# kkahatapitiya/Coarse-Fine-Networks

Hardware: AMD Instinct MI355X
Metric: clips/sec (fwd+bwd+SGD) x3d_fine X3D-M T=256x224x224 (higher is better)
Workload: dtype f32; 1 GPU; x3d_fine X3D-M train step (fwd+loss+bwd+SGD), 8x3x256x224x224 clips per GPU, random-init weights; clips_per_gpu=8, frames=256, parallelism=dp1, launch=eager

## Files before the change

coarse-fine-networks_amd/cfn_hip/ops.py:

```python
import torch
from torch.autograd import Function
from torch.autograd.function import once_differentiable

import ctypes
import threading

from . import call, call_try, check, query, last_error, ACT_NONE, ACT_RELU, ACT_SWISH, ACT_SIGMOID


_scratch_epoch = [0]


class _ZeroArena(object):
    CHUNK = 1 << 20

    def __init__(self):
        self.buf, self.off, self.epoch = {}, {}, _scratch_epoch[0]

    def take(self, numel, dev):
        if self.epoch != _scratch_epoch[0]:
            self.buf, self.off, self.epoch = {}, {}, _scratch_epoch[0]
        numel_al = (numel + 1) & ~1
        key = (dev.type, dev.index)
        if key not in self.buf or self.off[key] + numel_al > self.buf[key].numel():
            self.buf[key] = torch.zeros(max(self.CHUNK, numel_al), dtype=torch.float64, device=dev)
            self.off[key] = 0
        o = self.off[key]
        self.off[key] = o + numel_al
        return self.buf[key][o:o + numel]


class _GradCast(object):

    def __init__(self):
        self._reset()
        self.last_total = 0

    def _reset(self):
        self.cur, self.live, self.scheduled, self.seen, self.task = {}, [], False, set(), None

    def begin(self):
        tid = torch._C._current_graph_task_id()
        if tid != self.task:
            if self.live:
                self.flush()
            self._reset()
            self.task = tid

    def first_use(self, w):
        if id(w) in self.seen:
            return False
        self.seen.add(id(w))
        return True

    def take(self, numel, shape, dev):
        al = (numel + 3) & ~3
        key = (dev.type, dev.index)
        ch = self.cur.get(key)
        if ch is None or ch['off'] + al > ch['f64'].numel():
            size = max(int(self.last_total * 1.05) + 1024, al, 1 << 16)
            ch = {'f64': torch.zeros(size, dtype=torch.float64, device=dev),
                  'f32': torch.empty(size, dtype=torch.float32, device=dev), 'off': 0, 'done': 0}
            self.cur[key] = ch
            self.live.append(ch)
        o = ch['off']
        ch['off'] = o + al
        if not self.scheduled:
            torch.autograd.Variable._execution_engine.queue_callback(self._end_of_backward)
            self.scheduled = True
        return ch['f64'][o:o + numel], ch['f32'][o:o + numel].view(shape)

    def flush(self):
        for ch in self.live:
            if ch['off'] > ch['done']:
                ch['f32'][ch['done']:ch['off']].copy_(ch['f64'][ch['done']:ch['off']])
                ch['done'] = ch['off']

    def _end_of_backward(self):
        self.flush()
        self.last_total = max(sum(ch['off'] for ch in self.live), 1)
        self._reset()


class _PerThread(threading.local):

    def __init__(self):
        self.arena = _ZeroArena()
# ... 344 lines not shown


class _DwConvT5(Function):

    @staticmethod
    def forward(ctx, x, w, want_stats, out_dtype=None):
        x = check(x, torch.float32).contiguous()
        N, C, T, H, W = x.shape
        y = torch.empty_like(x, dtype=out_dtype or x.dtype)
        s = q = None
        if want_stats:
            s, q = _f64(N, C, x.device), _f64(N, C, x.device)
        w2 = w.reshape(C, 5).contiguous()
        call('cfn_dwconv_t5_fwd' + _sfx(y), x, w2, y, s, q, N, C, T, H * W)
        ctx.save_for_backward(x, w2, y)
        ctx.wshape = tuple(w.shape)
        ctx.wparam = w
        if not want_stats:
            return y, None, None
        return y, s, q

    @staticmethod
    @once_differentiable
    def backward(ctx, gy, gs, gq):
        x, w2, y = ctx.saved_tensors
        N, C, T, H, W = x.shape
        gy = torch.zeros_like(y) if gy is None else gy.contiguous()
        gs, gq = _opt(gs), _opt(gq)
        gx = gw = None
        want_x, want_w = ctx.needs_input_grad[0], ctx.needs_input_grad[1]
        if want_x:
            gx = torch.empty_like(x)
        if want_w:
            g64, fin = _gw_buffers(ctx.wparam, C, 5, x.device)
        fused = want_x and want_w and call_try('cfn_dwconv_t5_bwd_fused' + _sfx(y), gy, y, gs, gq, w2, x, gx, g64, N, C, T, H * W)
        if not fused:
            if want_x:
                call('cfn_dwconv_t5_bwd_data' + _sfx(y), gy, y, gs, gq, w2, gx, N, C, T, H * W)
            if want_w:
                call('cfn_dwconv_t5_bwd_weight' + _sfx(y), gy, y, gs, gq, x, g64, N, C, T, H * W)
        if want_w:
            gw = fin()
        return gx, gw, None, None


def dwconv_t5(x, w, stats=True, out_dtype=None):
    return _DwConvT5.apply(x, w, stats, out_dtype)


class _StemConv(Function):

    @staticmethod
    def forward(ctx, x, w):
        x = check(x).contiguous()
        N, Ci, T, H, W = x.shape
        Co = w.shape[0]
        Ho, Wo = (H + 2 - 3) // 2 + 1, (W + 2 - 3) // 2 + 1
        y = torch.empty(N, Co, T, Ho, Wo, dtype=torch.float32, device=x.device)
        w2 = w.reshape(Co, Ci * 9).contiguous()
        call('cfn_stem_conv_fwd', x, w2, y, N, Ci, Co, T, H, W)
        ctx.save_for_backward(x)
        ctx.wshape = tuple(w.shape)
        ctx.wparam = w
        return y

    @staticmethod
    @once_differentiable
    def backward(ctx, gy):
        (x,) = ctx.saved_tensors
        N, Ci, T, H, W = x.shape
        Co = ctx.wshape[0]
        gw = None
        if ctx.needs_input_grad[1]:
            g64, fin = _gw_buffers(ctx.wparam, Co, Ci * 9, x.device)
            call('cfn_stem_conv_bwd_weight', gy.contiguous(), x, g64, N, Ci, Co, T, H, W)
            gw = fin()
        return None, gw


def stem_conv(x, w):
    return _StemConv.apply(x, w)


from .u8clips import clip_lut


def _u8_args(frames, lengths, lut):
    if frames.dtype != torch.uint8 or frames.dim() != 5 or frames.shape[4] != 3:
        raise RuntimeError('uint8 frames of shape (N, T, H, W, 3) expected, got %s %s' % (frames.dtype, tuple(frames.shape)))
    if lut.dtype != torch.float32 or lut.numel() != 3 * 256:
        raise RuntimeError('a (3, 256) fp32 table expected (ops.clip_lut), got %s %s' % (lut.dtype, tuple(lut.shape)))
    if lengths is not None:
        if lengths.numel() != frames.shape[0]:
            raise RuntimeError('one length per clip expected: %d clips, lengths %s' % (frames.shape[0], tuple(lengths.shape)))
        lengths = lengths.to(torch.int32).contiguous()
    return frames.contiguous(), lengths, lut.contiguous()


def clip_u8_to_f32(frames, lut, lengths=None):
    frames, lengths, lut = _u8_args(frames, lengths, lut)
    N, T, H, W, _ = frames.shape
    x = torch.empty(N, 3, T, H, W, dtype=torch.float32, device=frames.device)
    call('cfn_clip_u8_to_f32', frames, lut, lengths, x, N, T, H, W)
    return x


class _StemConvU8(Function):

    @staticmethod
    def forward(ctx, frames, lengths, lut, w):
        frames, lengths, lut = _u8_args(frames, lengths, lut)
        N, T, H, W, Ci = frames.shape
        Co = w.shape[0]
        Ho, Wo = (H + 2 - 3) // 2 + 1, (W + 2 - 3) // 2 + 1
        y = torch.empty(N, Co, T, Ho, Wo, dtype=torch.float32, device=frames.device)
        w2 = w.reshape(Co, Ci * 9).contiguous()
        if not call_try('cfn_stem_conv_u8_fwd', frames, lut, lengths, w2, y, N, Ci, Co, T, H, W):
            call('cfn_stem_conv_fwd', clip_u8_to_f32(frames, lut, lengths), w2, y, N, Ci, Co, T, H, W)
        ctx.save_for_backward(frames, lengths, lut)
        ctx.wshape = tuple(w.shape)
        ctx.wparam = w
        return y

    @staticmethod
    @once_differentiable
    def backward(ctx, gy):
        frames, lengths, lut = ctx.saved_tensors
        N, T, H, W, Ci = frames.shape
        Co = ctx.wshape[0]
        gw = None
        if ctx.needs_input_grad[3]:
            g64, fin = _gw_buffers(ctx.wparam, Co, Ci * 9, frames.device)
            gy = gy.contiguous()
            if not call_try('cfn_stem_conv_u8_bwd_weight', gy, frames, lut, lengths, g64, N, Ci, Co, T, H, W):
                call('cfn_stem_conv_bwd_weight', gy, clip_u8_to_f32(frames, lut, lengths), g64, N, Ci, Co, T, H, W)
            gw = fin()
        return None, None, None, gw


def stem_conv_u8(frames, lengths, lut, w):
    return _StemConvU8.apply(frames, lengths, lut, w)


from . import u8aug

_AUG_TABLES = {}
_AUG_TABLES_MAX = 256


def aug_tables(box, size, device):
    cs = tuple(int(v) for v in box.detach().reshape(-1, 4)[:, 2].cpu().tolist())
    device = torch.device(device)
    key = (cs, int(size), device.type, device.index)
    hit = _AUG_TABLES.get(key)
    if hit is None:
        if any(c <= 0 or c > 4 * int(size) for c in cs):
            raise RuntimeError('crop_resize_flip_u8: crop extents %s into %d: 1 <= c <= 4 * size expected (the kernel takes tables of up '
                               'to %d taps; there is no CPU fallback)' % (sorted(set(cs)), size, u8aug.MAX_TAPS))
        bounds, coef = u8aug.batch_tables(cs, size)
        hit = (bounds.to(device), coef.to(device))
        if len(_AUG_TABLES) >= _AUG_TABLES_MAX:
            _AUG_TABLES.clear()
        _AUG_TABLES[key] = hit
    return hit


# ... 1185 lines not shown
```

coarse-fine-networks_amd/x3d_coarse.py:

```python
import threading

import torch
import torch.nn as nn
import torch.nn.functional as F

from cfn_hip import ops, ACT_NONE, ACT_RELU, ACT_SWISH, ACT_SIGMOID
from interp1d import Interp1d
from x3d_fine import (SubBatchNorm3d, Swish, Bottleneck, Deferred, conv3x3x3, conv1x1x1, _count,
                      get_inplanes, get_blocks)
import x3d_fine

FUSION_HW = 7


def _o():
    if x3d_fine.USE_TORCH_OPS:
        from cfn_hip import torchlib
        return torchlib.TorchOps
    return ops


def _w5(conv1d):
    w = conv1d.weight
    return w.view(w.shape[0], w.shape[1], 1, 1, 1)
# ... 248 lines not shown
        return mix(bias, self.conv_at, ACT_NONE), mix(scale, self.conv_at2, ACT_SIGMOID)

    def forward(self, inp):
        x, bias, scale = inp
        h = x.shape[3]
        zero = lambda v: torch.zeros(v.shape[1], device=v.device)
        down = lambda v: (v[:, :, :, ::v.shape[3] // FUSION_HW, ::v.shape[4] // FUSION_HW].contiguous(), zero(v))
        c7, m7 = self.forward7([down(v) for v in bias], [down(v) for v in scale])
        return _upsample(c7, h), _upsample(m7, h)


class _ZeroGradFor(torch.autograd.Function):

    @staticmethod
    def forward(ctx, t, param):
        ctx.meta = (tuple(param.shape), param.dtype, param.device)
        return t.view_as(t)

    @staticmethod
    def backward(ctx, g):
        shape, dt, dev = ctx.meta
        return g, torch.zeros(shape, dtype=dt, device=dev)


class GridPoolLayer(nn.Module):

    def __init__(self, ratio, depth):
        super(GridPoolLayer, self).__init__()
        self.ratio = 4
        self.depth = depth
        self.conv1 = nn.Conv3d(depth, depth, kernel_size=(3, 3, 3), stride=(self.ratio // 2, 2, 2), padding=1)
        self.bn1 = SubBatchNorm3d(num_splits=1, num_features=depth, affine=True)
        self.conv2 = nn.Conv3d(depth, depth, kernel_size=(3, 3, 3), stride=(self.ratio // 2, 2, 2), padding=1)
        self.bn2 = SubBatchNorm3d(num_splits=1, num_features=depth, affine=True)
        self.conv3 = nn.Conv3d(depth, 1, kernel_size=(1, 3, 3), stride=(1, 2, 2), padding=(0, 1, 1))
        self.relu = nn.ReLU(inplace=True)
        self.sigmoid = nn.Sigmoid()

    def _conv_bn(self, x, conv, bn, A, B, act):
        n = x.shape[0]
        st = tuple(conv.stride)
        y, s, q = _o().conv3d_dense(x, conv.weight, (3, 3, 3), st, (1, 1, 1), A, B, act, stats=self.training)
        A2, B2 = (bn.fold_op if x3d_fine.USE_TORCH_OPS else bn.fold)(s, q, _count(y), n)
        if not self.training:
            return y, A2, torch.addcmul(B2, A2, conv.bias.to(B2.dtype).view(1, -1))
        with torch.no_grad():
            bn.split_bn.running_mean.view(-1, bn.num_features).add_(conv.bias.view(1, -1), alpha=bn.momentum)
        return y, A2, _ZeroGradFor.apply(B2, conv.bias)

    def saliency(self, x):
        y1, A1, B1 = self._conv_bn(x, self.conv1, self.bn1, None, None, ACT_NONE)
        y2, A2, B2 = self._conv_bn(y1, self.conv2, self.bn2, A1, B1, ACT_RELU)
        y3, _, _ = _o().conv3d_dense(y2, self.conv3.weight, (1, 3, 3), (1, 2, 2), (0, 1, 1), A2, B2, ACT_RELU, stats=False)
        g = _o().pool_hw(y3, 1, 1)
        return g.view(g.shape[0], g.shape[2])

    @staticmethod
    def cdf(g, bias=None):
        return _o().grid_cdf(g, bias)

    def forward(self, inp):
        x = inp.materialize() if isinstance(inp, Deferred) else inp
        gx_out = self.cdf(self.saliency(x), self.conv3.bias)
        return _o().time_sample(x, gx_out), gx_out


def GridUnpool(inp, return_aux=False):
    x, gx, is_logit = inp
    ratio = 4
    b, k = gx.shape
    mid = torch.arange(k, device=gx.device).to(torch.float32)
    mid = (mid / (k - 1.)).view(1, -1).repeat(b, 1)
    gx_inv, ind = Interp1d().forward(gx, mid, mid, None, return_index=True)
    if is_logit:
        y = _o().time_sample(x.unsqueeze(3), gx_inv).squeeze(3)
    else:
        y = _o().time_resize(_o().time_sample(x, gx_inv), x.shape[2] * ratio)
    if return_aux:
        return y, gx_inv, ind
    return y


class ResNet(x3d_fine.ResNet):

    def __init__(self, block, layers, block_inplanes, n_input_channels=3, feat_depth={}, conv1_t_size=7,
                 conv1_t_stride=1, shortcut_type='B', widen_factor=1.0, dropout=0.5, n_classes=400, base_bn_splits=8,
                 task='class', extract_feat=False, t_pool=None, learnedMixing=False, isMixing=False, act_dtype=None):
        self.feat_depth, self.learnedMixing, self.isMixing, self.t_pool = feat_depth, learnedMixing, isMixing, t_pool
        nn.Module.__init__(self)
        planes = [(int(x * widen_factor), int(y * widen_factor)) for x, y in block_inplanes]
        if t_pool == 'avg':
            self.pool_1 = nn.AvgPool3d((4, 1, 1), stride=(4, 1, 1))
        elif t_pool == 'max':
            self.pool_1 = nn.MaxPool3d((4, 1, 1), stride=(4, 1, 1))
        elif t_pool == 'grid':
            self.pool_1 = GridPoolLayer(ratio=4, depth=planes[0][1])
        x3d_fine.ResNet.__init__(self, block, layers, block_inplanes, n_input_channels=n_input_channels,
                                 shortcut_type=shortcut_type, widen_factor=widen_factor, dropout=dropout,
                                 n_classes=n_classes, base_bn_splits=base_bn_splits, task=task,
                                 extract_feat=extract_feat, _skip_module_init=True, act_dtype=act_dtype)
        self.rw2 = RewightLayer(planes[0][1], planes[0][1], feat_depth['layer1'], 56)
        self.rw3 = RewightLayer(planes[1][1], planes[1][1], feat_depth['layer2'], 28)
        self.rw4 = RewightLayer(planes[2][1], planes[2][1], feat_depth['layer3'], 14)
        self.rw5 = RewightLayer(planes[3][1], planes[3][1], feat_depth['layer4'], 7)
        self.rw6 = RewightLayer(157, 157, feat_depth['conv5'], 7, pool=True)
        if self.isMixing:
            self.mix2 = MixingLayer(planes[0][1], learned=learnedMixing, index=0)
            self.mix3 = MixingLayer(planes[1][1], learned=learnedMixing, index=1)
            self.mix4 = MixingLayer(planes[2][1], learned=learnedMixing, index=2)
            self.mix5 = MixingLayer(planes[3][1], learned=learnedMixing, index=3)
        self.gauss = Gaussian(ratio=1)
        for m in self.modules():
            if isinstance(m, nn.Conv3d):
                nn.init.kaiming_normal_(m.weight, mode='fan_out', nonlinearity='relu')

    def replace_logits(self, n_classes):
        dev = self.fc1.weight.device
        self.fc2 = nn.Linear(2048, n_classes).to(dev)
        self.rw6 = RewightLayer(n_classes, n_classes, self.feat_depth['conv5'], 7, pool=True).to(dev)

    def forward(self, inp):
        x, feat, feat_masks, i, meta = inp
        tl = x.shape[2]
        x = self.layer1(self._stem(x))
        if self.act_dtype != torch.float32:
            x = (x.materialize() if isinstance(x, Deferred) else x).float()
        if self.t_pool == 'grid':
            x, gx = self.pool_1(x)
            GX = self.gauss([meta, feat_masks, gx, tl])
        else:
            if self.t_pool == 'stride':
                x = x[:, :, ::4].contiguous()
            elif self.t_pool in ('avg', 'max'):
                x = ops.time_pool(x.materialize() if isinstance(x, Deferred) else x, self.t_pool, 4)
            GX = self.gauss([meta, feat_masks, x, None])
        b2 = x.shape[0]
        levels = (('layer1', self.rw2), ('layer2', self.rw3), ('layer3', self.rw4), ('layer4', self.rw5))
        stages = (None, self.layer2, self.layer3, self.layer4)
        with _row_bank(b2, self._bias_groups(levels, feat, b2)):
            return self._fuse(x, feat, feat_masks, GX, gx if self.t_pool == 'grid' else None, b2, levels, stages)

    def _bias_groups(self, levels, feat, b2):
        rws = [m for _, m in levels] + ([] if self.extract_feat else [self.rw6])
        groups = []
        for m in rws:
            groups += [[m.fc1.bias]] + ([[m.fc3.bias]] if m.g_channels is not None else [])
        for (k, m) in list(levels) + ([] if self.extract_feat else [('conv5', self.rw6)]):
            if feat[k].shape[0] == b2:
                groups.append([m.at1.bias])
        if self.isMixing:
            groups += [[m.fc2.bias for _, m in levels], [m.fc4.bias for _, m in levels]]
            for mix in (self.mix2, self.mix3, self.mix4, self.mix5):
                if mix.learned:
                    groups += [[mix.conv_at.bias], [mix.conv_at2.bias]]
        else:
            for _, m in levels:
                groups += [[m.fc2.bias], [m.fc4.bias]]
        return groups

    def _fuse(self, x, feat, feat_masks, GX, gx, b2, levels, stages):
        if self.isMixing:
            rw = [m.forward7(feat[k], b2, feat_masks, GX, True) for k, m in levels]
            rb, rs = MixingLayer.prepare([r[0] for r in rw]), MixingLayer.prepare([r[1] for r in rw])
            for li, mix in enumerate((self.mix2, self.mix3, self.mix4, self.mix5)):
                if stages[li] is not None:
                    x = stages[li](x)
# ... 31 lines not shown
```

coarse-fine-networks_amd/x3d_fine.py:

```python
import os

import torch
import torch.nn as nn
import torch.nn.functional as F

from cfn_hip import ops, ACT_NONE, ACT_RELU, ACT_SWISH
from cfn_hip.u8clips import U8Clips

USE_TORCH_OPS = os.environ.get('CFN_USE_TORCH_OPS', '0') == '1'


class Deferred(object):
    __slots__ = ('raw', 'A', 'B', 'act')

    def __init__(self, raw, A, B, act):
        self.raw, self.A, self.B, self.act = raw, A, B, act

    @property
    def shape(self):
        return self.raw.shape

    def materialize(self):
        return ops.affine_act(self.raw, self.A, self.B, self.act)

# ... 198 lines not shown
            super(ResNet, self).__init__()
        block_inplanes = [(int(x * widen_factor), int(y * widen_factor)) for x, y in block_inplanes]
        self.index = 0
        self.base_bn_splits = base_bn_splits
        self.task = task
        self.extract_feat = extract_feat
        self.global_tower = global_tower
        self.t_downsample = t_downsample
        self.act_dtype = {None: torch.float32, 'f32': torch.float32, 'fp32': torch.float32, torch.float32: torch.float32,
                          'bf16': torch.bfloat16, torch.bfloat16: torch.bfloat16,
                          'fp16': torch.float16, 'f16': torch.float16, torch.float16: torch.float16}[act_dtype]
        self.in_planes = block_inplanes[0][1]

        self.conv1_s = nn.Conv3d(n_input_channels, self.in_planes, kernel_size=(1, 3, 3), stride=(1, 2, 2),
                                 padding=(0, 1, 1), bias=False)
        self.conv1_t = nn.Conv3d(self.in_planes, self.in_planes, kernel_size=(5, 1, 1), stride=(1, 1, 1),
                                 padding=(2, 0, 0), bias=False, groups=self.in_planes)
        self.bn1 = SubBatchNorm3d(num_splits=base_bn_splits, num_features=self.in_planes, affine=True)
        self.relu = nn.ReLU(inplace=True)
        self.layer1 = self._make_layer(block, block_inplanes[0], layers[0], shortcut_type, stride=2)
        self.layer2 = self._make_layer(block, block_inplanes[1], layers[1], shortcut_type, stride=2)
        self.layer3 = self._make_layer(block, block_inplanes[2], layers[2], shortcut_type, stride=2)
        self.layer4 = self._make_layer(block, block_inplanes[3], layers[3], shortcut_type, stride=2)
        self.conv5 = nn.Conv3d(block_inplanes[3][1], block_inplanes[3][0], kernel_size=(1, 1, 1), stride=(1, 1, 1),
                               padding=(0, 0, 0), bias=False)
        self.bn5 = SubBatchNorm3d(num_splits=base_bn_splits, num_features=block_inplanes[3][0], affine=True)
        if task == 'class':
            self.avgpool = nn.AdaptiveAvgPool3d((1, 1, 1))
        elif task == 'loc':
            self.avgpool = nn.AdaptiveAvgPool3d((None, 1, 1))
        self.fc1 = nn.Conv3d(block_inplanes[3][0], 2048, bias=False, kernel_size=1, stride=1)
        self.fc2 = nn.Linear(2048, n_classes)
        self.dropout = nn.Dropout(dropout)

        for m in self.modules():
            if isinstance(m, nn.Conv3d):
                nn.init.kaiming_normal_(m.weight, mode='fan_out', nonlinearity='relu')

    def _make_layer(self, block, planes, blocks, shortcut_type, stride=1):
        downsample = None
        if stride != 1 or self.in_planes != planes[1]:
            if shortcut_type == 'A':
                downsample = ('A', planes[1], stride)
            else:
                downsample = nn.Sequential(
                    conv1x1x1(self.in_planes, planes[1], stride, t_downsample=self.t_downsample),
                    SubBatchNorm3d(num_splits=self.base_bn_splits, num_features=planes[1], affine=True))
        layers = [block(in_planes=self.in_planes, planes=planes, stride=stride, downsample=downsample,
                        index=self.index, base_bn_splits=self.base_bn_splits, t_downsample=self.t_downsample)]
        self.in_planes = planes[1]
        self.index += 1
        for _ in range(1, blocks):
            layers.append(block(self.in_planes, planes, index=self.index, base_bn_splits=self.base_bn_splits,
                                t_downsample=self.t_downsample))
            self.index += 1
        self.index = 0
        for blk in layers[:-1]:
            blk.split_out = True
        return nn.Sequential(*layers)

    def replace_logits(self, n_classes):
        self.fc2 = nn.Linear(2048, n_classes).to(self.fc1.weight.device)

    def update_bn_splits_long_cycle(self, long_cycle_bn_scale):
        for m in self.modules():
            if isinstance(m, SubBatchNorm3d):
                m.num_splits = self.base_bn_splits * long_cycle_bn_scale
                m.split_bn = nn.BatchNorm3d(num_features=m.num_features * m.num_splits, affine=False).to(m.weight.device)
        return self.base_bn_splits * long_cycle_bn_scale

    def aggregate_sub_bn_stats(self):
        count = 0
        for m in self.modules():
            if isinstance(m, SubBatchNorm3d):
                m.aggregate_stats()
                count += 1
        return count

    def set_input_norm(self, mean, std, norm_value=255):
        lut = ops.clip_lut(mean, std, norm_value).to(self.conv1_s.weight.device)
        self.register_buffer('input_lut', lut, persistent=False)
        return self

    def _conv1_s(self, x):
        if not isinstance(x, U8Clips):
            return ops.stem_conv(x, self.conv1_s.weight)
        lut = getattr(self, 'input_lut', None)
        if lut is None:
            raise RuntimeError('the model was handed uint8 frames (U8Clips) but does not know how to normalise them: call '
                               'set_input_norm(mean, std) first (e.g. CHARADES_MEAN / CHARADES_STD)')
        if x.frames.dim() != 5:
            raise RuntimeError('U8Clips of shape (N, T, H, W, 3) expected (flatten_crops() a collated batch), got %s'
                               % (tuple(x.frames.shape),))
        return ops.stem_conv_u8(x.frames, x.lengths, lut, self.conv1_s.weight)

    def _stem(self, x):
        y = self._conv1_s(x)
        y, s, q = ops.dwconv_t5(y, self.conv1_t.weight, stats=self.training, out_dtype=self.act_dtype)
        A, B = self.bn1.fold(s, q, _count(y), y.shape[0])
        return Deferred(y, A, B, ACT_RELU)

    def _head(self, x):
        n = x.shape[0]
        y5, s5, q5 = ops.pwconv(x, self.conv5.weight, stats=self.training)
        A5, B5 = self.bn5.fold(s5, q5, _count(y5), n)
        if self.task == 'class':
            pooled = ops.pool_hw(y5, 1, 1, A5, B5, ACT_RELU).mean(dim=2, keepdim=True)
        else:
            pooled = ops.pool_hw(y5, 1, 1, A5, B5, ACT_RELU)
        if self.extract_feat:
            return pooled
        f1, _, _ = ops.pwconv(pooled, self.fc1.weight, stats=False)
        one = torch.ones(n, f1.shape[1], device=f1.device)
        z = ops.affine_act(f1, one, torch.zeros_like(one), ACT_RELU)
        z = self.dropout(z)
        out, _, _ = ops.pwconv(z, self.fc2.weight.view(self.fc2.weight.shape[0], -1, 1, 1, 1), stats=False)
        out = out.squeeze(4).squeeze(3) + self.fc2.bias.view(1, -1, 1)
        return out

    def forward(self, inp):
        x, masks = inp
        x = self._stem(x)
        feat_g = {}
        for i, layer in enumerate((self.layer1, self.layer2, self.layer3, self.layer4), start=1):
            x = layer(x)
            if self.global_tower:
                feat_g['layer%d' % i] = ops.pool_hw(x, 7, 7)
        if self.global_tower:
            n = x.shape[0]
            y5, s5, q5 = ops.pwconv(x, self.conv5.weight, stats=self.training)
            A5, B5 = self.bn5.fold(s5, q5, _count(y5), n)
            feat_g['conv5'] = ops.pool_hw(y5, 7, 7, A5, B5, ACT_RELU)
            return feat_g, masks
        return self._head(x)


def replace_logits(self, n_classes):
    self.fc2 = nn.Linear(2048, n_classes)


def get_inplanes(version):
    planes = {'S': [(54, 24), (108, 48), (216, 96), (432, 192)],
              'M': [(54, 24), (108, 48), (216, 96), (432, 192)],
              'XL': [(72, 32), (162, 72), (306, 136), (630, 280)]}
    return planes[version]


def get_blocks(version):
    blocks = {'S': [3, 5, 11, 7], 'M': [3, 5, 11, 7], 'XL': [5, 10, 25, 15]}
    return blocks[version]


def generate_model(x3d_version, **kwargs):
    return ResNet(Bottleneck, get_blocks(x3d_version), get_inplanes(x3d_version), **kwargs)
```

include/cfn_hip.h:

```cpp
#ifndef CFN_HIP_H
#define CFN_HIP_H
#ifdef __cplusplus
extern "C" {
#endif

const char* cfn_last_error(void);
const char* cfn_version(void);
int cfn_device_info(int* cus, int* lds_per_cu, char* name, int name_len);

int cfn_prof_enable(int family, int on);
int cfn_prof_collect(int family, double* total_ms, long* launches, double* total_bytes);

int cfn_dwconv3d_fwd(const float* x, const double* A, const double* B, int act, const float* w, float* y, double* sum,
                     double* sumsq, int N, int C, int T, int Hi, int Wi, int stride, void* stream);
int cfn_dwconv3d_bwd_data(const float* gy, const float* y, const double* gsum, const double* gsumsq, const float* w,
                          const float* x, const double* A, const double* B, int act, float* gx, double* gA, double* gB,
                          int N, int C, int T, int Hi, int Wi, int stride, void* stream);
int cfn_dwconv3d_bwd_weight(const float* gy, const float* y, const double* gsum, const double* gsumsq, const float* x,
                            const double* A, const double* B, int act, double* gw, int N, int C, int T, int Hi, int Wi,
                            int stride, void* stream);
int cfn_dwconv3d_bwd_fused(const float* gy, const float* y, const double* gsum, const double* gsumsq, const float* w,
                           const float* x, const double* A, const double* B, int act, float* gx, double* gA, double* gB,
                           double* gw, int N, int C, int T, int H, int W, void* stream);
int cfn_dwconv3d_bwd_fused_s2(const float* gy, const float* y, const double* gsum, const double* gsumsq, const float* w,
                              const float* x, const double* A, const double* B, int act, float* gx, double* gA, double* gB,
                              double* gw, int N, int C, int T, int H, int W, void* stream);

int cfn_dwconv_t5_fwd(const float* x, const float* w, float* y, double* sum, double* sumsq, int N, int C, int T,
                      long plane, void* stream);
int cfn_dwconv_t5_bwd_data(const float* gy, const float* y, const double* gsum, const double* gsumsq, const float* w,
                           float* gx, int N, int C, int T, long plane, void* stream);
int cfn_dwconv_t5_bwd_weight(const float* gy, const float* y, const double* gsum, const double* gsumsq, const float* x,
                             double* gw, int N, int C, int T, long plane, void* stream);
int cfn_dwconv_t5_bwd_fused(const float* gy, const float* y, const double* gsum, const double* gsumsq, const float* w,
                            const float* x, float* gx, double* gw, int N, int C, int T, long plane, void* stream);

int cfn_pwconv_fwd(const float* x, const double* A, const double* B, int act, const float* w, float* y, double* sum,
                   double* sumsq, int N, int Cin, int Cout, int T, int Hi, int Wi, int stride, void* stream);
int cfn_pwconv_bwd_data(const float* gy, const float* y, const double* gsum, const double* gsumsq, const float* w,
                        const float* x, const double* A, const double* B, int act, float* gx, double* gA, double* gB, int N,
                        int Cin, int Cout, int T, int Hi, int Wi, int stride, void* stream);
int cfn_pwconv_bwd_data_acc(const float* gy, const float* y, const double* gsum, const double* gsumsq, const float* w,
                        const float* x, const double* A, const double* B, int act, float* gx, double* gA, double* gB, int N,
                        int Cin, int Cout, int T, int Hi, int Wi, int stride, const float* acc, int acc_stride,
                        const double* gscale, void* stream);
int cfn_pwconv_bwd_weight(const float* gy, const float* y, const double* gsum, const double* gsumsq, const float* x,
                          const double* A, const double* B, int act, double* gw, int N, int Cin, int Cout, int T, int Hi,
                          int Wi, int stride, const double* gscale, void* stream);

int cfn_pw_split_terms(int terms);

int cfn_pwconv_route(int op, int N, int Cin, int Cout, int T, int Hi, int Wi, int stride, int act, int flags, char* out, int cap);

int cfn_deterministic(int on);

int cfn_pwconv_bwd_fused(const float* gy, const float* y, const double* gsum, const double* gsumsq, const float* w,
                         const float* x, const double* A, const double* B, int act, float* gx, double* gA, double* gB,
                         double* gw, int N, int Cin, int Cout, int T, int Hi, int Wi, const float* acc, int acc_stride,
                         const double* gscale, void* stream);

int cfn_pwconv_short_bwd(const float* gy, const float* y, const double* gsum, const double* gsumsq, const double* gscale,
                         const float* w, const float* x, const double* A, const double* B, int act, float* da, double* gw,
                         int N, int Cin, int Cout, int T, int Hi, int Wi, int stride, void* stream);

int cfn_stem_conv_fwd(const float* x, const float* w, float* y, int N, int Cimg, int Cout, int T, int Hi, int Wi,
                      void* stream);
int cfn_stem_conv_bwd_weight(const float* gy, const float* x, double* gw, int N, int Cimg, int Cout, int T, int Hi, int Wi,
                             void* stream);

int cfn_clip_u8_to_f32(const unsigned char* frames, const float* lut, const int* lengths, float* x, int N, int T, int H, int W,
                       void* stream);
int cfn_stem_conv_u8_fwd(const unsigned char* frames, const float* lut, const int* lengths, const float* w, float* y, int N,
                         int Cimg, int Cout, int T, int Hi, int Wi, void* stream);
int cfn_stem_conv_u8_bwd_weight(const float* gy, const unsigned char* frames, const float* lut, const int* lengths, double* gw,
                                int N, int Cimg, int Cout, int T, int Hi, int Wi, void* stream);

int cfn_bn_fold_fwd(const double* s, const double* q, const float* gamma, const float* beta, float* run_mean, float* run_var,
                    long* nbt, int training, int N, int C, int S, double count, double eps, double momentum, const float* w1,
                    const float* b1, const float* w2, const float* b2, int Wd, double pool_count, double* A, double* B,
                    double* mean, double* rstd, float* A0, float* B0, float* gate, float* hbuf, float* pooled, void* stream);
int cfn_bn_fold_bwd(const double* gA, const double* gB, const double* s, const float* gamma, const double* mean,
                    const double* rstd, const float* A0, const float* B0, const float* gate, const float* hbuf,
                    const float* pooled, const float* w1, const float* w2, int training, int N, int C, int S, int Wd,
                    double count, double pool_count, double* gs, double* gq, float* ggamma, float* gbeta, float* gw1,
                    float* gb1, float* gw2, float* gb2, double* tA, double* tB, void* stream);

int cfn_conv3d_dense_fwd(const float* x, const double* A, const double* B, int act, const float* w, float* y, double* sum,
                         double* sumsq, int N, int Cin, int Cout, int T, int Hi, int Wi, const int* geom, void* stream);
int cfn_conv3d_dense_bwd_data(const float* gy, const float* y, const double* gsum, const double* gsumsq, const float* w,
                              const float* x, const double* A, const double* B, int act, float* gx, double* gA, double* gB,
                              int N, int Cin, int Cout, int T, int Hi, int Wi, const int* geom, void* stream);
int cfn_conv3d_dense_bwd_weight(const float* gy, const float* y, const double* gsum, const double* gsumsq, const float* x,
                                const double* A, const double* B, int act, double* gw, int N, int Cin, int Cout, int T, int Hi,
                                int Wi, const int* geom, void* stream);

int cfn_gauss_align_fwd(const long* meta, const float* mask, const float* gx, double tx, double ratio, float* GX, int B, int crops,
                        int Tf, int K, void* stream);
int cfn_gauss_align_bwd(const float* gGX, const long* meta, const float* mask, const float* gx, double tx, double ratio,
                        float* ggx, int B, int crops, int Tf, int K, void* stream);

int cfn_fusion_gather_fwd(const float* x, const float* at_raw, const float* at_bias, const float* GX, const float* mask, float* z,
                          float* den, int B, int crops, int C, int Tf, int K, int P, void* stream);
int cfn_fusion_gather_bwd(const float* gz, const float* z, const float* den, const float* x, const float* at_raw,
                          const float* at_bias, const float* GX, const float* mask, float* gx, float* gat, float* gGX, float* dw,
                          int B, int crops, int C, int Tf, int K, int P, void* stream);

int cfn_bn_add_relu_fwd(const float* y, const double* A, const double* B, const float* res, const double* Ar, const double* Br,
                        float* out, int* mask, long NC, long vol, void* stream);
int cfn_bn_add_relu_bwd(const float* gout, const float* gout2, const float* out, const float* y, const double* A, const float* res,
                        const double* Ar, float* gy, float* gres, double* gA, double* gB, double* gAr, long NC, long vol,
                        void* stream);
long cfn_bn_add_relu_mask_words(long NC, long vol);
int cfn_bn_add_relu_bwd_g(const float* gout, const float* gout2, const float* out, const int* mask, const float* y,
                          const float* res, float* g, double* gA, double* gB, double* gAr, long NC, long vol, void* stream);

int cfn_affine_act_fwd(const float* x, const double* A, const double* B, int act, float* out, long NC, long vol, void* stream);
int cfn_affine_act_bwd(const float* gout, const float* x, const double* A, const double* B, int act, float* gx, double* gA,
                       double* gB, long NC, long vol, void* stream);
int cfn_channel_stats(const float* x, double* sum, double* sumsq, long NC, long vol, void* stream);

int cfn_pool_hw_fwd(const float* x, const double* A, const double* B, int act, float* out, long NC, int T, int H, int W, int OH,
                    int OW, void* stream);
int cfn_pool_hw_bwd(const float* gout, const float* x, const double* A, const double* B, int act, float* gx, double* gA,
                    double* gB, long NC, int T, int H, int W, int OH, int OW, void* stream);

int cfn_film_fwd(const float* x, const float* m, const float* c, float* out, long NC, int T, int H, int W, int f,
                 void* stream);
int cfn_film_bwd(const float* g, const float* x, const float* m, float* gx, float* gm, float* gc, long NC, int T, int H,
                 int W, int f, void* stream);

int cfn_grid_time_index(const float* cdf, int n, int Tin, int* i0, float* w1, void* stream);
int cfn_grid_cdf_fwd(const float* g, const float* bias, float* cdf, int B, int Kin, void* stream);
int cfn_grid_cdf_bwd(const float* gcdf, const float* g, const float* bias, float* gg, int B, int Kin, void* stream);
int cfn_time_sample_fwd(const float* x, const float* cdf, float* out, int B, int C, int Tin, int K, long P, void* stream);
int cfn_time_sample_bwd(const float* g, const float* x, const float* cdf, float* gx, double* gcdf, int B, int C, int Tin,
                        int K, long P, void* stream);

int cfn_time_pool_fwd(const float* x, float* out, int mode, long BC, int Tin, int R, long P, void* stream);
int cfn_time_pool_bwd(const float* g, const float* x, float* gx, int mode, long BC, int Tin, int R, long P, void* stream);

int cfn_interp1d_fwd(const float* x, const float* y, const float* xnew, float* ynew, long* ind, int B, int N, int Pq,
                     int xrow, int yrow, int qrow, void* stream);
int cfn_interp1d_bwd(const float* g, const float* x, const float* y, const float* xnew, const long* ind, float* gx, float* gy,
                     float* gq, int B, int N, int Pq, int xrow, int yrow, int qrow, void* stream);

int cfn_time_resize_fwd(const float* x, float* out, long BC, int Kin, int Lout, long P, int align_corners, void* stream);
int cfn_time_resize_bwd(const float* g, float* gx, long BC, int Kin, int Lout, long P, int align_corners, void* stream);

int cfn_detloss_fwd(const float* logits, const float* labels, const float* masks, const float* norm, double world, float* probs,
                    float* cls, float* loc, int* jstar, float* ymax, double* rows, double* norm_used, int B, int C, int T, int TL,
                    int n, int align_corners, void* stream);
// ... 173 lines not shown
```

Baseline: 106.6 clips/s.

## Fuse stem spatial conv and temporal depthwise conv into paired fwd/bwd kernels

Adds stem_pair forward and backward HIP kernels that compute the 3x3 stride-2 stem conv with MFMA and feed it straight into the 5-tap temporal depthwise conv with BN statistics, all in one pass over banded tiles held in LDS. The backward kernel folds the depthwise-conv data gradient directly into the stem weight-gradient MFMA accumulation, so the intermediate gradient tensor is never written to global memory. The goal is to cut the kernel launches and the large intermediate-tensor round trips at full 112x112 resolution. In exchange the code is specialised to 3->24 channels at 224x224, falls back to the old path otherwise, and still writes xs for backward.

Result: faster. 108.4 clips/s (median of 6 runs) (+1.7%).

```diff
diff --git a/coarse-fine-networks_amd/cfn_hip/ops.py b/coarse-fine-networks_amd/cfn_hip/ops.py
--- a/coarse-fine-networks_amd/cfn_hip/ops.py
+++ b/coarse-fine-networks_amd/cfn_hip/ops.py
@@ -3,6 +3,7 @@
 from torch.autograd.function import once_differentiable
 
 import ctypes
+import os
 import threading
 
 from . import call, call_try, check, query, last_error, ACT_NONE, ACT_RELU, ACT_SWISH, ACT_SIGMOID
@@ -513,6 +514,79 @@
     return _StemConv.apply(x, w)
 
 
+def _stem_pair_switch():
+    try:
+        return int(os.environ.get('CFN_STEM_PAIR', '3'))
+    except ValueError:
+        raise RuntimeError('CFN_STEM_PAIR must be an integer (bit 0: forward, bit 1: backward), got %r' % os.environ['CFN_STEM_PAIR'])
+
+
+class _StemPair(Function):
+
+    @staticmethod
+    def forward(ctx, x, w_s, w_t, want_stats, run_frames):
+        x = check(x).contiguous()
+        if x.dtype != torch.float32:
+            raise RuntimeError('stem_pair: fp32 clip expected, got %s' % x.dtype)
+        N, Ci, T, H, W = x.shape
+        Co = w_s.shape[0]
+        Ho, Wo = (H + 2 - 3) // 2 + 1, (W + 2 - 3) // 2 + 1
+        xs = torch.empty(N, Co, T, Ho, Wo, dtype=torch.float32, device=x.device)
+        y = torch.empty_like(xs)
+        s = q = None
+        if want_stats:
+            s, q = _f64(N, Co, x.device), _f64(N, Co, x.device)
+        ws2 = w_s.reshape(Co, Ci * 9).contiguous()
+        wt2 = w_t.reshape(Co, 5).contiguous()
+        if not (_stem_pair_switch() & 1 and call_try('cfn_stem_pair_fwd', x, ws2, wt2, xs, y, s, q, N, Ci, Co, T, H, W, run_frames)):
+            call('cfn_stem_conv_fwd', x, ws2, xs, N, Ci, Co, T, H, W)
+            call('cfn_dwconv_t5_fwd', xs, wt2, y, s, q, N, Co, T, Ho * Wo)
+        ctx.save_for_backward(x, xs, y, wt2)
+        ctx.params = (w_s, w_t)
+        ctx.run_frames = run_frames
+        if not want_stats:
+            return y, None, None
+        return y, s, q
+
+    @staticmethod
+    @once_differentiable
+    def backward(ctx, gy, gs, gq):
+        x, xs, y, wt2 = ctx.saved_tensors
+        w_s, w_t = ctx.params
+        N, Ci, T, H, W = x.shape
+        _, Co, _, Ho, Wo = xs.shape
+        gy = torch.zeros_like(y) if gy is None else gy.contiguous()
+        gs, gq = _opt(gs), _opt(gq)
+        want_s, want_t = ctx.needs_input_grad[1], ctx.needs_input_grad[2]
+        gws = gwt = None
+        if want_s and want_t:
+            gs64, fin_s = _gw_buffers(w_s, Co, Ci * 9, x.device)
+            gt64, fin_t = _gw_buffers(w_t, Co, 5, x.device)
+            if not (_stem_pair_switch() & 2 and
+                    call_try('cfn_stem_pair_bwd', gy, y, gs, gq, wt2, xs, x, gt64, gs64, N, Ci, Co, T, H, W, ctx.run_frames)):
+                gxs = torch.empty_like(xs)
+                if not call_try('cfn_dwconv_t5_bwd_fused', gy, y, gs, gq, wt2, xs, gxs, gt64, N, Co, T, Ho * Wo):
+                    call('cfn_dwconv_t5_bwd_data', gy, y, gs, gq, wt2, gxs, N, Co, T, Ho * Wo)
+                    call('cfn_dwconv_t5_bwd_weight', gy, y, gs, gq, xs, gt64, N, Co, T, Ho * Wo)
+                call('cfn_stem_conv_bwd_weight', gxs, x, gs64, N, Ci, Co, T, H, W)
+            gws, gwt = fin_s(), fin_t()
+        elif want_t:
+            gt64, fin_t = _gw_buffers(w_t, Co, 5, x.device)
+            call('cfn_dwconv_t5_bwd_weight', gy, y, gs, gq, xs, gt64, N, Co, T, Ho * Wo)
+            gwt = fin_t()
+        elif want_s:
+            gs64, fin_s = _gw_buffers(w_s, Co, Ci * 9, x.device)
+            gxs = torch.empty_like(xs)
+            call('cfn_dwconv_t5_bwd_data', gy, y, gs, gq, wt2, gxs, N, Co, T, Ho * Wo)
+            call('cfn_stem_conv_bwd_weight', gxs, x, gs64, N, Ci, Co, T, H, W)
+            gws = fin_s()
+        return None, gws, gwt, None, None
+
+
+def stem_pair(x, w_s, w_t, stats=True, run_frames=0):
+    return _StemPair.apply(x, w_s, w_t, stats, run_frames)
+
+
 from .u8clips import clip_lut
 
 
diff --git a/coarse-fine-networks_amd/csrc/stempair.hip b/coarse-fine-networks_amd/csrc/stempair.hip
--- /dev/null
+++ b/coarse-fine-networks_amd/csrc/stempair.hip
@@ -0,0 +1,425 @@
+#include "cfn_common.h"
+#include <stdlib.h>
+
+typedef float __attribute__((ext_vector_type(16))) sp16;
+typedef float __attribute__((ext_vector_type(4))) sp4;
+typedef float __attribute__((ext_vector_type(2))) sp2;
+
+struct StemPairBwdArgs {
+    const float* gy; const float* y; const double* gs; const double* gq; const float* wt; const float* xs; const float* x;
+    double* gwt; double* gws;
+    int N, T, R, nch, runs, per_block;
+};
+
+namespace {
+constexpr int SP_WI = 224, SP_WO = 112, SP_RB = 2, SP_RIN = 2 * SP_RB + 1, SP_PITCH = 228;
+constexpr int SP_CIS = SP_RIN * SP_PITCH + 24;
+constexpr int SP_GP = 2 * SP_WO + 2;
+constexpr int SP_P = SP_WI * SP_WI, SP_PO = SP_WO * SP_WO, SP_BANDS = SP_WO / SP_RB, SP_OOB = 0x7fff0000;
+constexpr int SP_XU = 3 * SP_RIN * (SP_WI / 4), SP_NXU = (SP_XU + 511) / 512;
+constexpr int SP_GU = 24 * SP_RB * (SP_WO / 4), SP_NGU = (SP_GU + 511) / 512;
+constexpr int SP_UPC = SP_RB * (SP_WO / 4);
+
+struct SpCur {
+    int run, n, band, ta, tb, t;
+    __device__ __forceinline__ void start(int r, int R, int nch, int T) {
+        run = r;
+        band = r % SP_BANDS;
+        const int q = r / SP_BANDS, chunk = q % nch;
+        n = q / nch;
+        ta = chunk * R;
+        tb = min(ta + R, T);
+        t = ta - 4;
+    }
+    __device__ __forceinline__ void next(int R, int nch, int T) {
+        if (++t == tb) start(run + 1, R, nch, T);
+    }
+};
+}
+
+__device__ __forceinline__ float sp_taps(float a0, float a1, float a2, float a3, float a4, float w0, float w1, float w2, float w3, float w4) {
+    return __builtin_fmaf(a4, w4, __builtin_fmaf(a3, w3, __builtin_fmaf(a2, w2, __builtin_fmaf(a0, w0, __fmul_rn(a1, w1)))));
+}
+
+template <bool HASY>
+__global__ __launch_bounds__(512) void stem_pair_bwd_kernel(const StemPairBwdArgs a) {
+    __shared__ __attribute__((aligned(16))) float lds[3 * SP_CIS + 24 * SP_GP];
+    float* const img = lds;
+    float* const gbuf = lds + 3 * SP_CIS;
+    const int tid = threadIdx.x, lane = tid & 63, wave = cfn_uni(tid >> 6), h = lane >> 5, p = lane & 31;
+    const int T = a.T, R = a.R, nch = a.nch;
+
+    for (int i = tid; i < 3 * SP_CIS; i += 512) img[i] = 0.0f;
+
+    int xo[SP_NXU], xl[SP_NXU], xr[SP_NXU];
+#pragma unroll
+    for (int k = 0; k < SP_NXU; ++k) {
+        const int e = k * 512 + tid;
+        const int rowid = e / (SP_WI / 4), c4 = e - rowid * (SP_WI / 4), ci = rowid / SP_RIN, r = rowid - ci * SP_RIN;
+        const bool in = e < SP_XU;
+        xo[k] = in ? (int)(((long)ci * T * SP_P + (long)r * SP_WI + c4 * 4) * 4) : SP_OOB;
+        xl[k] = in ? ci * SP_CIS + r * SP_PITCH + 4 + c4 * 4 : -1;
+        xr[k] = r;
+    }
+    int go[SP_NGU], gl[SP_NGU], gc[SP_NGU];
+    float wk[SP_NGU][5];
+#pragma unroll
+    for (int k = 0; k < SP_NGU; ++k) {
+        const int e = k * 512 + tid;
+        const int co = e / SP_UPC, rem = e - co * SP_UPC;
+        const bool in = e < SP_GU;
+        go[k] = in ? (int)(((long)co * T * SP_PO + rem * 4) * 4) : SP_OOB;
+        gl[k] = in ? co * SP_GP + rem * 4 : -1;
+        gc[k] = in ? co : 0;
+#pragma unroll
+        for (int j = 0; j < 5; ++j) wk[k][j] = a.wt[gc[k] * 5 + 4 - j];
+    }
+    const int ohl = wave >> 2, ow0 = (wave & 3) * 28;
+    const int colp = p < 27 ? p : 0;
+    const int ci = colp / 9, kh = (colp - ci * 9) / 3, kw = colp - ci * 9 - kh * 3;
+    const float* bp = img + ci * SP_CIS + (2 * ohl + kh) * SP_PITCH + 2 * ow0 + kw + 3 + 2 * h;
+    const float* ap = gbuf + min(p, 23) * SP_GP + ohl * SP_WO + ow0 + h;
+
+    sp16 acc0, acc1;
+#pragma unroll
+    for (int r = 0; r < 16; ++r) acc0[r] = acc1[r] = 0.0f;
+    float acct[SP_NGU][5];
+#pragma unroll
+    for (int k = 0; k < SP_NGU; ++k)
+#pragma unroll
+        for (int j = 0; j < 5; ++j) acct[k][j] = 0.0f;
+
+    const int first = (int)cfn_xcd_remap(blockIdx.x, gridDim.x) * a.per_block, last = min(first + a.per_block, a.runs);
+    const unsigned gbytes = (unsigned)((long)24 * T * SP_PO * 4), xbytes = (unsigned)((long)3 * T * SP_P * 4);
+    sp4 fg[SP_NGU], fy[SP_NGU], fs[SP_NGU], fx[SP_NXU];
+    auto fetch = [&](const SpCur& c) {
+        const bool on = c.run < last;
+        const int n = on ? c.n : 0, f = c.t + 2;
+        const bool fv = on && f >= 0 && f < T, xv = on && c.t >= c.ta;
+        __amdgpu_buffer_rsrc_t rg = cfn_rsrc(a.gy + (long)n * 24 * T * SP_PO, gbytes);
+        __amdgpu_buffer_rsrc_t ry = cfn_rsrc((HASY ? a.y : a.gy) + (long)n * 24 * T * SP_PO, gbytes);
+        __amdgpu_buffer_rsrc_t rs = cfn_rsrc(a.xs + (long)n * 24 * T * SP_PO, gbytes);
+        __amdgpu_buffer_rsrc_t rx = cfn_rsrc(a.x + (long)n * 3 * T * SP_P, xbytes);
+        const int ih0 = 2 * c.band * SP_RB - 1;
+        const int sg = cfn_uni(fv ? (f * SP_PO + c.band * SP_RB * SP_WO) * 4 : 0);
+        const int ss = cfn_uni(xv ? (c.t * SP_PO + c.band * SP_RB * SP_WO) * 4 : 0);
+        const int sx = cfn_uni(xv ? c.t * SP_P * 4 : 0), rowoff = cfn_uni(ih0 * SP_WI * 4);
+#pragma unroll
+        for (int k = 0; k < SP_NGU; ++k) {
+            fg[k] = __builtin_bit_cast(sp4, __builtin_amdgcn_raw_buffer_load_b128(rg, fv ? go[k] : SP_OOB, sg, 0));
+            if (HASY) fy[k] = __builtin_bit_cast(sp4, __builtin_amdgcn_raw_buffer_load_b128(ry, fv ? go[k] : SP_OOB, sg, 0));
+        }
+#pragma unroll
+        for (int k = 0; k < SP_NGU; ++k)
+            fs[k] = __builtin_bit_cast(sp4, __builtin_amdgcn_raw_buffer_load_b128(rs, xv ? go[k] : SP_OOB, ss, 0));
+#pragma unroll
+        for (int k = 0; k < SP_NXU; ++k)
+            fx[k] = __builtin_bit_cast(sp4, __builtin_amdgcn_raw_buffer_load_b128(rx, (xv && xo[k] != SP_OOB && ih0 + xr[k] >= 0) ? xo[k] + rowoff : SP_OOB, sx, 0));
+    };
+
+    const sp4 zero = {0.f, 0.f, 0.f, 0.f};
+    sp4 W[5][SP_NGU];
+#pragma unroll
+    for (int i = 0; i < 5; ++i)
+#pragma unroll
+        for (int k = 0; k < SP_NGU; ++k) W[i][k] = zero;
+    float gsv[SP_NGU], gqv[SP_NGU];
+#pragma unroll
+    for (int k = 0; k < SP_NGU; ++k) gsv[k] = gqv[k] = 0.0f;
+
+    SpCur cc, fc;
+    cc.start(first, R, nch, T);
+    fc = cc;
+    __syncthreads();
+    fetch(fc);
+    fc.next(R, nch, T);
+    while (cc.run < last) {
+        if (cc.t == cc.ta - 4) {
+#pragma unroll
+            for (int k = 0; k < SP_NGU; ++k) {
+                gsv[k] = a.gs ? (float)a.gs[cc.n * 24 + gc[k]] : 0.0f;
+                gqv[k] = (HASY && a.gq) ? 2.0f * (float)a.gq[cc.n * 24 + gc[k]] : 0.0f;
+            }
+        }
+        const bool mm = cc.t >= cc.ta;
+        const float m = (cc.t + 2 >= 0 && cc.t + 2 < T) ? 1.0f : 0.0f;
+#pragma unroll
+        for (int k = 0; k < SP_NGU; ++k) {
+            sp4 v = fg[k] + gsv[k];
+            if (HASY) v = __builtin_elementwise_fma(fy[k], (sp4){gqv[k], gqv[k], gqv[k], gqv[k]}, v);
+            W[4][k] = v * m;
+        }
+        if (mm) {
+#pragma unroll
+            for (int k = 0; k < SP_NGU; ++k) {
+                sp4 gx;
+#pragma unroll
+                for (int i = 0; i < 4; ++i)
+                    gx[i] = sp_taps(W[0][k][i], W[1][k][i], W[2][k][i], W[3][k][i], W[4][k][i], wk[k][0], wk[k][1], wk[k][2], wk[k][3], wk[k][4]);
+                if (gl[k] >= 0) {
+                    *reinterpret_cast<sp2*>(gbuf + gl[k]) = (sp2){gx.x, gx.y};
+                    *reinterpret_cast<sp2*>(gbuf + gl[k] + 2) = (sp2){gx.z, gx.w};
+                }
+#pragma unroll
+                for (int j = 0; j < 5; ++j) {
+                    const sp4 pr = fs[k] * W[4 - j][k];
+                    acct[k][j] += (pr.x + pr.y) + (pr.z + pr.w);
+                }
+            }
+#pragma unroll
+            for (int k = 0; k < SP_NXU; ++k)
+                if (xl[k] >= 0) *reinterpret_cast<sp4*>(img + xl[k]) = fx[k];
+            __syncthreads();
+        }
+        fetch(fc);
+        fc.next(R, nch, T);
+        if (mm) {
+#pragma unroll
+            for (int j = 0; j < 14; j += 2) {
+                acc0 = __builtin_amdgcn_mfma_f32_32x32x2f32(ap[2 * j], bp[4 * j], acc0, 0, 0, 0);
+                acc1 = __builtin_amdgcn_mfma_f32_32x32x2f32(ap[2 * j + 2], bp[4 * j + 4], acc1, 0, 0, 0);
+            }
+            __syncthreads();
+        }
+#pragma unroll
+        for (int i = 0; i < 4; ++i)
+#pragma unroll
+            for (int k = 0; k < SP_NGU; ++k) W[i][k] = W[i + 1][k];
+        cc.next(R, nch, T);
+    }
+
+    __syncthreads();
+#pragma unroll
+    for (int k = 0; k < SP_NGU; ++k)
+        if (gl[k] >= 0) {
+#pragma unroll
+            for (int j = 0; j < 5; ++j) lds[(k * 512 + tid) * 5 + j] = acct[k][j];
+        }
+    __syncthreads();
+    if (tid < 24 * 5) {
+        const int co = tid / 5, j = tid - co * 5;
+        float s = 0.0f;
+        for (int u = 0; u < SP_UPC; ++u) s += lds[(co * SP_UPC + u) * 5 + j];
+        cfn_add64(&a.gwt[co * 5 + j], (double)s);
+    }
+    __syncthreads();
+#pragma unroll
+    for (int r = 0; r < 16; ++r) lds[(wave * 16 + r) * 64 + lane] = acc0[r] + acc1[r];
+    __syncthreads();
+    for (int e = tid; e < 16 * 64; e += 512) {
+        const int r = e >> 6, l = e & 63, hh = l >> 5, col = l & 31;
+        const int co = (r & 3) + 8 * (r >> 2) + 4 * hh;
+        float s = 0.0f;
+#pragma unroll
+        for (int w = 0; w < 8; ++w) s += lds[(w * 16 + r) * 64 + l];
+        if (co < 24 && col < 27) cfn_add64(&a.gws[co * 27 + col], (double)s);
+    }
+}
+
+static int stem_pair_plan(int N, int T, int wgs) {
+    int best = T;
+    long best_cost = -1;
+    for (int nch = 1; nch == 1 || T / nch >= 32; ++nch) {
+        const int R = cfn_cdiv(T, nch);
+        const long runs = (long)N * cfn_cdiv(T, R) * SP_BANDS, per = (runs + wgs - 1) / wgs, cost = per * (R + 2);
+        if (best_cost < 0 || cost < best_cost) { best_cost = cost; best = R; }
+    }
+    return best;
+}
+
+static int stem_pair_cus() {
+    static int cus = 0;
+    if (!cus) { int dev = 0; hipDeviceProp_t pr; cus = (hipGetDevice(&dev) == hipSuccess && hipGetDeviceProperties(&pr, dev) == hipSuccess) ? pr.multiProcessorCount : 256; }
+    return cus;
+}
+
+static bool stem_pair_shape_ok(int Cimg, int Cout, int T, int Hi, int Wi) {
+    return Cimg == 3 && Cout == 24 && Hi == SP_WI && Wi == SP_WI && (long)24 * T * SP_PO * 4 < 0x7fff0000L;
+}
+
+extern "C" int cfn_stem_pair_bwd(const float* gy, const float* y, const double* gsum, const double* gsumsq, const float* w_t, const float* xs,
+                                 const float* x, double* gw_t, double* gw_s, int N, int Cimg, int Cout, int T, int Hi, int Wi, int run_frames,
+                                 void* stream) {
+    CFN_REQUIRE(gy && w_t && xs && x && gw_t && gw_s, "cfn_stem_pair_bwd: null tensor");
+    CFN_REQUIRE(gsumsq == nullptr || y != nullptr, "cfn_stem_pair_bwd: gsumsq needs y");
+    CFN_REQUIRE(N > 0 && Cimg > 0 && Cout > 0 && T > 0 && Hi > 0 && Wi > 0 && run_frames >= 0, "cfn_stem_pair_bwd: bad shape");
+    if (!stem_pair_shape_ok(Cimg, Cout, T, Hi, Wi)) return -1;
+    const bool hasy = y != nullptr && gsumsq != nullptr;
+    if ((((uintptr_t)gy | (uintptr_t)xs | (uintptr_t)x | (uintptr_t)(hasy ? y : gy)) & 15) != 0) return -1;
+    const int wgs = stem_pair_cus();
+    const int R = run_frames > 0 ? (run_frames < T ? run_frames : T) : stem_pair_plan(N, T, wgs);
+    const int nch = cfn_cdiv(T, R);
+    const long runs = (long)N * nch * SP_BANDS;
+    if (runs >= (1L << 30)) return -1;
+    long blocks = runs < wgs ? runs : wgs;
+    const long per = (runs + blocks - 1) / blocks;
+    blocks = (runs + per - 1) / per;
+    StemPairBwdArgs a = {gy, hasy ? y : nullptr, gsum, hasy ? gsumsq : nullptr, w_t, xs, x, gw_t, gw_s, N, T, R, nch, (int)runs, (int)per};
+    hipStream_t st = (hipStream_t)stream;
+    CfnProfScope prof(CFN_K_STEM, st, 4.0 * N * T * ((double)3 * SP_P + (double)24 * SP_PO * (hasy ? 3 : 2)));
+    if (hasy) hipLaunchKernelGGL(stem_pair_bwd_kernel<true>, dim3((unsigned)blocks), dim3(512), 0, st, a);
+    else hipLaunchKernelGGL(stem_pair_bwd_kernel<false>, dim3((unsigned)blocks), dim3(512), 0, st, a);
+    return cfn_check_launch("stem_pair_bwd");
+}
+
+static constexpr __host__ __device__ int sp_tap(int k) { return k < 27 ? (k / 9) * SP_CIS + ((k % 9) / 3) * SP_PITCH + k % 3 : 0; }
+
+struct StemPairFwdArgs {
+    const float* x; const float* ws; const float* wt; float* xs; float* y; double* s1; double* s2;
+    int N, T, R, nch, runs;
+};
+
+__global__ __launch_bounds__(448, 4) void stem_pair_fwd_kernel(const StemPairFwdArgs a) {
+    constexpr int NT = 448, NXU = (SP_XU + NT - 1) / NT, KP = 14;
+    __shared__ __attribute__((aligned(16))) float img[2][3 * SP_CIS];
+    __shared__ __attribute__((aligned(16))) float wts[24 * 8];
+    __shared__ float wsl[14 * 64];
+    __shared__ float red[2][7][24];
+    const int tid = threadIdx.x, lane = tid & 63, wave = cfn_uni(tid >> 6), half = lane >> 5, col = lane & 31;
+    const int T = a.T;
+    SpCur c;
+    c.start((int)cfn_xcd_remap(blockIdx.x, gridDim.x), a.R, a.nch, T);
+    const int n = c.n, band = c.band, ta = c.ta, tb = c.tb;
+
+    for (int i = tid; i < 2 * 3 * SP_CIS; i += NT) (&img[0][0])[i] = 0.0f;
+    if (tid < 24 * 5) wts[(tid / 5) * 8 + tid % 5] = a.wt[tid];
+
+    const int ih0 = 2 * band * SP_RB - 1;
+    int xo[NXU], xl[NXU];
+#pragma unroll
+    for (int k = 0; k < NXU; ++k) {
+        const int e = k * NT + tid;
+        const int rowid = e / (SP_WI / 4), c4 = e - rowid * (SP_WI / 4), ci = rowid / SP_RIN, r = rowid - ci * SP_RIN;
+        const bool in = e < SP_XU;
+        xo[k] = (in && ih0 + r >= 0) ? (int)(((long)ci * T * SP_P + (long)(ih0 + r) * SP_WI + c4 * 4) * 4) : SP_OOB;
+        xl[k] = in ? ci * SP_CIS + r * SP_PITCH + 4 + c4 * 4 : -1;
+    }
+    if (wave == 0) {
+#pragma unroll
+        for (int s = 0; s < KP; ++s) {
+            const int k = 2 * s + half;
+            wsl[s * 64 + lane] = (k < 27 && col < 24) ? a.ws[col * 27 + k] : 0.0f;
+        }
+    }
+    const int pos = wave * 32 + col, ohl = pos / SP_WO, ow = pos - ohl * SP_WO;
+    const int lboff = 2 * ohl * SP_PITCH + 2 * ow + 3;
+
+    const unsigned gbytes = (unsigned)((long)24 * T * SP_PO * 4), xbytes = (unsigned)((long)3 * T * SP_P * 4);
+    __amdgpu_buffer_rsrc_t rx = cfn_rsrc(a.x + (long)n * 3 * T * SP_P, xbytes);
+    __amdgpu_buffer_rsrc_t rs = cfn_rsrc(a.xs + (long)n * 24 * T * SP_PO, gbytes);
+    __amdgpu_buffer_rsrc_t ry = cfn_rsrc(a.y + (long)n * 24 * T * SP_PO, gbytes);
+    const int vout = (half * 4 * T * SP_PO + band * SP_RB * SP_WO + pos) * 4;
+
+    sp4 fx[NXU];
+    auto fetch = [&](int s) {
+        const bool fv = s >= 0 && s < T && s <= tb + 1;
+        const int sx = cfn_uni(fv ? s * SP_P * 4 : 0);
+#pragma unroll
+        for (int k = 0; k < NXU; ++k)
+            fx[k] = __builtin_bit_cast(sp4, __builtin_amdgcn_raw_buffer_load_b128(rx, fv ? xo[k] : SP_OOB, sx, 0));
+    };
+    auto put = [&](int b) {
+#pragma unroll
+        for (int k = 0; k < NXU; ++k)
+            if (xl[k] >= 0) *reinterpret_cast<sp4*>(&img[b][xl[k]]) = fx[k];
+    };
+
+    float W[5][12], st1[12], st2[12];
+#pragma unroll
+    for (int r = 0; r < 12; ++r) {
+        st1[r] = st2[r] = 0.0f;
+#pragma unroll
+        for (int i = 0; i < 5; ++i) W[i][r] = 0.0f;
+    }
+
+    fetch(ta - 2);
+    __syncthreads();
+    put(0);
+    fetch(ta - 1);
+    __syncthreads();
+    int b = 0;
+    for (int s = ta - 2; s <= tb + 1; ++s, b ^= 1) {
+        put(b ^ 1);
+        fetch(s + 2);
+        const float* lb = &img[b][lboff];
+        int hsel = half;
+        asm volatile("" : "+v"(hsel));
+        sp16 acc;
+#pragma unroll
+        for (int r = 0; r < 16; ++r) acc[r] = 0.0f;
+#pragma unroll
+        for (int k = 0; k < KP; ++k) acc = __builtin_amdgcn_mfma_f32_32x32x2f32(wsl[k * 64 + lane], lb[hsel ? sp_tap(2 * k + 1) : sp_tap(2 * k)], acc, 0, 0, 0);
+        const bool own = s >= ta && s < tb, emit = s - 2 >= ta;
+#pragma unroll
+        for (int r = 0; r < 12; ++r) {
+            const int cr = (r & 3) + 8 * (r >> 2);
+            W[4][r] = acc[r];
+            __builtin_amdgcn_raw_buffer_store_b32(__builtin_bit_cast(unsigned, W[4][r]), rs, own ? vout : SP_OOB, cfn_uni(own ? (cr * T + s) * SP_PO * 4 : 0), 0);
+        }
+        if (emit) {
+#pragma unroll
+            for (int r = 0; r < 12; ++r) {
+                const int cr = (r & 3) + 8 * (r >> 2);
+                const float* wk = wts + (cr + 4 * half) * 8;
+                const float yv = sp_taps(W[0][r], W[1][r], W[2][r], W[3][r], W[4][r], wk[0], wk[1], wk[2], wk[3], wk[4]);
+                __builtin_amdgcn_raw_buffer_store_b32(__builtin_bit_cast(unsigned, yv), ry, vout, cfn_uni((cr * T + s - 2) * SP_PO * 4), 0);
+                st1[r] += yv;
+                st2[r] += yv * yv;
+            }
+        }
+#pragma unroll
+        for (int i = 0; i < 4; ++i)
+#pragma unroll
+            for (int r = 0; r < 12; ++r) W[i][r] = W[i + 1][r];
+        __syncthreads();
+    }
+    if (a.s1) {
+#pragma unroll
+        for (int r = 0; r < 12; ++r) {
+#pragma unroll
+            for (int o = 16; o > 0; o >>= 1) { st1[r] += __shfl_xor(st1[r], o, 64); st2[r] += __shfl_xor(st2[r], o, 64); }
+            if (col == 0) {
+                const int co = (r & 3) + 8 * (r >> 2) + 4 * half;
+                red[0][wave][co] = st1[r];
+                red[1][wave][co] = st2[r];
+            }
+        }
+        __syncthreads();
+        if (tid < 48) {
+            const int which = tid / 24, co = tid - which * 24;
+            float v = 0.0f;
+#pragma unroll
+            for (int w = 0; w < 7; ++w) v += red[which][w][co];
+            cfn_add64((which ? a.s2 : a.s1) + n * 24 + co, (double)v);
+        }
+    }
+}
+
+static int stem_pair_fwd_plan(int N, int T, int slots) {
+    int best = T;
+    long best_cost = -1;
+    for (int nch = 1; nch == 1 || T / nch >= 32; ++nch) {
+        const int R = cfn_cdiv(T, nch);
+        const long runs = (long)N * cfn_cdiv(T, R) * SP_BANDS, rounds = (runs + slots - 1) / slots, cost = rounds * (R + 4);
+        if (best_cost < 0 || cost < best_cost) { best_cost = cost; best = R; }
+    }
+    return best;
+}
+
+extern "C" int cfn_stem_pair_fwd(const float* x, const float* w_s, const float* w_t, float* xs, float* y, double* sum, double* sumsq, int N,
+                                 int Cimg, int Cout, int T, int Hi, int Wi, int run_frames, void* stream) {
+    CFN_REQUIRE(x && w_s && w_t && xs && y, "cfn_stem_pair_fwd: null tensor");
+    CFN_REQUIRE((sum == nullptr) == (sumsq == nullptr), "cfn_stem_pair_fwd: sum/sumsq mismatch");
+    CFN_REQUIRE(N > 0 && Cimg > 0 && Cout > 0 && T > 0 && Hi > 0 && Wi > 0 && run_frames >= 0, "cfn_stem_pair_fwd: bad shape");
+    if (!stem_pair_shape_ok(Cimg, Cout, T, Hi, Wi)) return -1;
+    if ((((uintptr_t)x | (uintptr_t)xs | (uintptr_t)y) & 15) != 0) return -1;
+    const int R = run_frames > 0 ? (run_frames < T ? run_frames : T) : stem_pair_fwd_plan(N, T, 2 * stem_pair_cus());
+    const int nch = cfn_cdiv(T, R);
+    const long runs = (long)N * nch * SP_BANDS;
+    if (runs >= (1L << 30)) return -1;
+    StemPairFwdArgs a = {x, w_s, w_t, xs, y, sum, sumsq, N, T, R, nch, (int)runs};
+    hipStream_t st = (hipStream_t)stream;
+    CfnProfScope prof(CFN_K_STEM, st, 4.0 * N * T * ((double)3 * SP_P + (double)24 * SP_PO * 2));
+    hipLaunchKernelGGL(stem_pair_fwd_kernel, dim3((unsigned)runs), dim3(448), 0, st, a);
+    return cfn_check_launch("stem_pair_fwd");
+}
diff --git a/coarse-fine-networks_amd/x3d_coarse.py b/coarse-fine-networks_amd/x3d_coarse.py
--- a/coarse-fine-networks_amd/x3d_coarse.py
+++ b/coarse-fine-networks_amd/x3d_coarse.py
@@ -354,6 +354,8 @@
 
 
 class ResNet(x3d_fine.ResNet):
+
+    FUSED_STEM_PAIR = False
 
     def __init__(self, block, layers, block_inplanes, n_input_channels=3, feat_depth={}, conv1_t_size=7,
                  conv1_t_stride=1, shortcut_type='B', widen_factor=1.0, dropout=0.5, n_classes=400, base_bn_splits=8,
diff --git a/coarse-fine-networks_amd/x3d_fine.py b/coarse-fine-networks_amd/x3d_fine.py
--- a/coarse-fine-networks_amd/x3d_fine.py
+++ b/coarse-fine-networks_amd/x3d_fine.py
@@ -304,6 +304,8 @@
         self.register_buffer('input_lut', lut, persistent=False)
         return self
 
+    FUSED_STEM_PAIR = True
+
     def _conv1_s(self, x):
         if not isinstance(x, U8Clips):
             return ops.stem_conv(x, self.conv1_s.weight)
@@ -317,8 +319,11 @@
         return ops.stem_conv_u8(x.frames, x.lengths, lut, self.conv1_s.weight)
 
     def _stem(self, x):
-        y = self._conv1_s(x)
-        y, s, q = ops.dwconv_t5(y, self.conv1_t.weight, stats=self.training, out_dtype=self.act_dtype)
+        if self.FUSED_STEM_PAIR and isinstance(x, torch.Tensor) and x.dtype == torch.float32 and self.act_dtype == torch.float32 and not USE_TORCH_OPS:
+            y, s, q = ops.stem_pair(x, self.conv1_s.weight, self.conv1_t.weight, stats=self.training)
+        else:
+            y = self._conv1_s(x)
+            y, s, q = ops.dwconv_t5(y, self.conv1_t.weight, stats=self.training, out_dtype=self.act_dtype)
         A, B = self.bn1.fold(s, q, _count(y), y.shape[0])
         return Deferred(y, A, B, ACT_RELU)
 
diff --git a/include/cfn_hip.h b/include/cfn_hip.h
--- a/include/cfn_hip.h
+++ b/include/cfn_hip.h
@@ -67,6 +67,12 @@
                       void* stream);
 int cfn_stem_conv_bwd_weight(const float* gy, const float* x, double* gw, int N, int Cimg, int Cout, int T, int Hi, int Wi,
                              void* stream);
+
+int cfn_stem_pair_fwd(const float* x, const float* w_s, const float* w_t, float* xs, float* y, double* sum, double* sumsq, int N,
+                      int Cimg, int Cout, int T, int Hi, int Wi, int run_frames, void* stream);
+int cfn_stem_pair_bwd(const float* gy, const float* y, const double* gsum, const double* gsumsq, const float* w_t, const float* xs,
+                      const float* x, double* gw_t, double* gw_s, int N, int Cimg, int Cout, int T, int Hi, int Wi, int run_frames,
+                      void* stream);
 
 int cfn_clip_u8_to_f32(const unsigned char* frames, const float* lut, const int* lengths, float* x, int N, int T, int H, int W,
                        void* stream);
```
